# Improbable-AI/walk-these-ways

Measured on NVIDIA H100. Metric: env_steps_per_s, higher is better.
Workload: dtype tf32

## Files before the change

walk-these-ways_b200/csrc/gemm_tf32.cu:

```cuda
#include <cuda_runtime.h>
#include <cuda.h>
#include <cuda_bf16.h>
#include <stdint.h>
#include <stdio.h>
#include <mutex>
#include <unordered_map>
#include <stdlib.h>
#include "../../include/go1_b200.h"
#include "wgmma_tf32.cuh"
#include "activation.cuh"

extern int go1_set_error(const char* m);
void go1_count_launch(int n);

namespace {

constexpr int BM = 128, BK = 32;
constexpr int NCONS = 8, EPI_G = 2;

__device__ __forceinline__ uint32_t smem_u32(const void* p) { return (uint32_t)__cvta_generic_to_shared(p); }

__device__ __forceinline__ void mbar_init(uint64_t* bar, uint32_t count) {
    asm volatile("mbarrier.init.shared::cta.b64 [%0], %1;" ::"r"(smem_u32(bar)), "r"(count));
}
__device__ __forceinline__ void mbar_expect_tx(uint64_t* bar, uint32_t bytes) {
    asm volatile("mbarrier.arrive.expect_tx.shared::cta.b64 _, [%0], %1;" ::"r"(smem_u32(bar)), "r"(bytes) : "memory");
}
__device__ __forceinline__ void mbar_wait(uint64_t* bar, uint32_t parity) {
    uint32_t done = 0;
    const uint32_t a = smem_u32(bar);
    while (!done) {
        asm volatile("{\n\t.reg .pred p;\n\tmbarrier.try_wait.parity.shared::cta.b64 p, [%1], %2;\n\tselp.u32 %0, 1, 0, p;\n\t}"
                     : "=r"(done) : "r"(a), "r"(parity) : "memory");
    }
}
__device__ __forceinline__ void mbar_arrive(uint64_t* bar) {
    asm volatile("mbarrier.arrive.shared::cta.b64 _, [%0];" ::"r"(smem_u32(bar)) : "memory");
}
__device__ __forceinline__ bool elect_one() {
    uint32_t pred = 0;
    asm volatile("{\n\t.reg .pred p;\n\telect.sync _|p, 0xffffffff;\n\tselp.u32 %0, 1, 0, p;\n\t}" : "=r"(pred));
    return pred != 0;
}
__device__ __forceinline__ void tma_load_2d(const CUtensorMap* map, uint64_t* bar, void* dst, int c0, int c1) {
    asm volatile("cp.async.bulk.tensor.2d.shared::cluster.global.mbarrier::complete_tx::bytes [%0], [%1, {%3, %4}], [%2];"
                 ::"r"(smem_u32(dst)), "l"(map), "r"(smem_u32(bar)), "r"(c0), "r"(c1) : "memory");
}
__device__ __forceinline__ void tma_load_2d_multicast(const CUtensorMap* map, uint64_t* bar, void* dst, int c0, int c1, uint16_t cta_mask) {
    asm volatile("cp.async.bulk.tensor.2d.shared::cluster.global.mbarrier::complete_tx::bytes.multicast::cluster [%0], [%1, {%3, %4}], [%2], %5;"
                 ::"r"(smem_u32(dst)), "l"(map), "r"(smem_u32(bar)), "r"(c0), "r"(c1), "h"(cta_mask) : "memory");
}
__device__ __forceinline__ uint32_t cluster_ctarank() {
    uint32_t r;
    asm("mov.u32 %0, %%cluster_ctarank;" : "=r"(r));
    return r;
}
__device__ __forceinline__ void cluster_sync() {
    asm volatile("barrier.cluster.arrive.release;\n\tbarrier.cluster.wait.acquire;" ::: "memory");
}
__device__ __forceinline__ void mbar_arrive_cluster(uint64_t* bar, uint32_t rank) {
    uint32_t remote;
    asm volatile("mapa.shared::cluster.u32 %0, %1, %2;" : "=r"(remote) : "r"(smem_u32(bar)), "r"(rank));
    asm volatile("mbarrier.arrive.shared::cluster.b64 _, [%0];" ::"r"(remote) : "memory");
}
__device__ __forceinline__ void cons_sync() { asm volatile("bar.sync 1, 256;" ::: "memory"); }
__device__ __forceinline__ void wg_sync(int wgi) { asm volatile("bar.sync %0, 128;" ::"r"(2 + wgi) : "memory"); }
__device__ __forceinline__ void fence_async_smem() { asm volatile("fence.proxy.async.shared::cta;" ::: "memory"); }

template <int W>
__device__ __forceinline__ void transpose_tile(const float* __restrict__ raw, uint8_t* dst, const int ctid) {
#pragma unroll
    for (int it = 0; it < W * 8 / 256; it++) {
        const int idx = ctid + 256 * it;
        const int mn = idx % W, kq = idx / W;
        const float* r = raw + (size_t)(4 * kq) * W + mn;
        *reinterpret_cast<float4*>(dst + mn * 128 + ((kq ^ (mn & 7)) << 4)) = make_float4(r[0], r[W], r[2 * W], r[3 * W]);
    }
}

template <int NJ, typename F>
__device__ __forceinline__ void store_fragment(const float (&acc)[4 * NJ], uint8_t* tile, const int col_base, const int w, const int lane, F f) {
    const int rb = 16 * w + (lane >> 2);
#pragma unroll
    for (int j = 0; j < NJ; j++) {
        const int col = col_base + 8 * j + 2 * (lane & 3);
        uint8_t* p = tile + (size_t)(col >> 5) * (64 * 128) + rb * 128 + ((((col & 31) >> 2) ^ (rb & 7)) << 4) + (lane & 1) * 8;
        *reinterpret_cast<float2*>(p) = f(make_float2(acc[4 * j], acc[4 * j + 1]), col, 0);
        *reinterpret_cast<float2*>(p + 8 * 128) = f(make_float2(acc[4 * j + 2], acc[4 * j + 3]), col, 1);
    }
}


struct GemmArgs {
    float* C; const float* bias;
    int M, N, K, ldc, act, kind, accumulate, kb_per_split;
    const float* ex; const float* wex; const float* aux;
    int ldex, ldwex, nex, ldaux;
    int lead;
    int amn, bmn;
    int ct;
    int c16;
    float* colsum;
    const float* bx; const float* bwx; float* gwx; float* dx;
    int ldbx, ldbwx, ldgwx, lddx, nbx;
    int tma_store, tma_aux;
    float* Cg[4]; int nprob, tiles_per_prob;
};
constexpr int GEMM_MAXP = 4;
struct GemmMaps { CUtensorMap a[GEMM_MAXP], b[GEMM_MAXP], half; };

struct EpiStage {
    uint8_t* out;
    const CUtensorMap* mapC;
    const uint8_t* aux;
};
__device__ __forceinline__ void tma_store_2d(const CUtensorMap* map, const void* src, int c0, int c1) {
    asm volatile("cp.async.bulk.tensor.2d.global.shared::cta.bulk_group [%0, {%2, %3}], [%1];"
                 ::"l"(map), "r"(smem_u32(src)), "r"(c0), "r"(c1) : "memory");
}

__device__ __forceinline__ uint32_t pack_bf16x2(float lo, float hi) {
    return (uint32_t)__bfloat16_as_ushort(__float2bfloat16_rn(lo)) | ((uint32_t)__bfloat16_as_ushort(__float2bfloat16_rn(hi)) << 16);
}

template <typename D>
__device__ __forceinline__ void epilogue_dact(const D dact, const GemmArgs& g, float (&v)[32], const int row, const int col0, const int ncols, const int lane,
                                              const float4 (&ypre)[8], const bool have_pre, const EpiStage& es) {
    const float* arow = g.aux + (size_t)row * g.ldaux + col0;
    if (es.aux) {
        const uint8_t* srow = es.aux + lane * 128;
#pragma unroll
        for (int j = 0; j < 8; j++) {
            const float4 y = *reinterpret_cast<const float4*>(srow + ((j ^ (lane & 7)) << 4));
            v[4 * j] *= dact(y.x); v[4 * j + 1] *= dact(y.y); v[4 * j + 2] *= dact(y.z); v[4 * j + 3] *= dact(y.w);
        }
    } else if (have_pre) {
#pragma unroll
        for (int j = 0; j < 8; j++) {
            const float4 y = ypre[j];
            v[4 * j] *= dact(y.x); v[4 * j + 1] *= dact(y.y); v[4 * j + 2] *= dact(y.z); v[4 * j + 3] *= dact(y.w);
        }
    } else if (ncols == 32 && (g.ldaux & 3) == 0 && ((((uintptr_t)g.aux) & 15) == 0) && ((col0 & 3) == 0)) {
#pragma unroll
        for (int j = 0; j < 8; j++) {
            const float4 y = __ldg(reinterpret_cast<const float4*>(arow) + j);
            v[4 * j] *= dact(y.x); v[4 * j + 1] *= dact(y.y); v[4 * j + 2] *= dact(y.z); v[4 * j + 3] *= dact(y.w);
        }
    } else {
#pragma unroll
        for (int j = 0; j < 32; j++) if (j < ncols) v[j] *= dact(__ldg(arow + j));
    }
}
// ... 56 lines not shown
            wl[t] = (t < g.nex && lead_j) ? __ldg(g.wex + (size_t)cj * g.ldwex + t) : 0.f;
        }
        if (g.nex <= 2) {
#pragma unroll
            for (int j = 0; j < 32; j++)
                v[j] += fmaf(e[1], __shfl_sync(0xffffffffu, wl[1], j), e[0] * __shfl_sync(0xffffffffu, wl[0], j));
        } else {
#pragma unroll
            for (int j = 0; j < 32; j++) {
                float a = e[0] * __shfl_sync(0xffffffffu, wl[0], j);
                a = fmaf(e[1], __shfl_sync(0xffffffffu, wl[1], j), a);
                a = fmaf(e[2], __shfl_sync(0xffffffffu, wl[2], j), a);
                v[j] += fmaf(e[3], __shfl_sync(0xffffffffu, wl[3], j), a);
            }
        }
    }
    if (g.bias) {
        const float bl = cj < g.N ? __ldg(g.bias + cj) : 0.f;
#pragma unroll
        for (int j = 0; j < 32; j++) v[j] += __shfl_sync(0xffffffffu, bl, j);
    }
    const int kind = ANYKIND ? g.kind : (int)GO1_ACT_ELU;
    if (row_ok) {
    if (g.act == 1) {
        const int nlead = g.lead <= 0 ? 32 : max(0, min(32, g.lead - col0));
        GO1_ACT_SWITCH(kind, KD,
            _Pragma("unroll")
            for (int j = 0; j < 32; j++) if (j < nlead) v[j] = act_fast<KD>(v[j]);)
    } else if (g.act == 2) {
        if (ANYKIND) epilogue_dact(act_deriv_coefficients(kind), g, v, row, col0, ncols, lane, ypre, have_pre, es);
        else epilogue_dact([](float y) { return act_deriv<GO1_ACT_ELU>(y); }, g, v, row, col0, ncols, lane, ypre, have_pre, es);
    }
    }
    if (g.colsum) {
        float sred[32];
#pragma unroll
        for (int j = 0; j < 32; j++) sred[j] = (row_ok && j < ncols) ? v[j] : 0.f;
        const float s = transpose_reduce32(sred, lane);
        if (lane < ncols) atomicAdd(g.colsum + col0 + lane, s);
    }
    if (g.nbx > 0) {
        const int cjx = col0 + lane;
#pragma unroll
        for (int t = 0; t < 4; t++) {
            if (t < g.nbx) {
                if (g.gwx) {
                const float e = row_ok ? __ldg(g.bx + (size_t)row * g.ldbx + t) : 0.f;
                float sred[32];
#pragma unroll
                for (int j = 0; j < 32; j++) sred[j] = (row_ok && j < ncols) ? v[j] * e : 0.f;
                const float s = transpose_reduce32(sred, lane);
                if (lane < ncols) atomicAdd(g.gwx + (size_t)cjx * g.ldgwx + t, s);
                }
                if (g.dx) {
                    const float wl = lane < ncols ? __ldg(g.bwx + (size_t)cjx * g.ldbwx + t) : 0.f;
                    float acc = 0.f;
#pragma unroll
                    for (int j = 0; j < 32; j++) acc = fmaf(v[j], __shfl_sync(0xffffffffu, wl, j), acc);
                    if (row_ok) atomicAdd(g.dx + (size_t)row * g.lddx + t, acc);
                }
            }
        }
    }
    if (ROW16 && g.c16 && !g.ct) {
        if (es.out) {
            __syncwarp();
            uint8_t* srow = es.out + lane * 64;
#pragma unroll
            for (int j = 0; j < 4; j++) {
                uint4 o;
                o.x = pack_bf16x2(v[8 * j], v[8 * j + 1]); o.y = pack_bf16x2(v[8 * j + 2], v[8 * j + 3]);
                o.z = pack_bf16x2(v[8 * j + 4], v[8 * j + 5]); o.w = pack_bf16x2(v[8 * j + 6], v[8 * j + 7]);
                *reinterpret_cast<uint4*>(srow + ((j ^ ((lane >> 1) & 3)) << 4)) = o;
            }
            asm volatile("fence.proxy.async.shared::cta;" ::: "memory");
            __syncwarp();
            if (lane == 0) {
                tma_store_2d(es.mapC, es.out, col0, row);
                asm volatile("cp.async.bulk.commit_group;" ::: "memory");
            }
        } else if (row_ok) {
            uint16_t* c16 = reinterpret_cast<uint16_t*>(Cbase) + (size_t)row * g.ldc + col0;
#pragma unroll
            for (int j = 0; j < 32; j++) if (j < ncols) c16[j] = __bfloat16_as_ushort(__float2bfloat16_rn(v[j]));
        }
        return;
    }
    if (es.out) {
        if (g.ct && g.c16) {
            __syncwarp();
#pragma unroll
            for (int j = 0; j < 32; j++) *reinterpret_cast<__nv_bfloat16*>(es.out + j * 64 + lane * 2) = __float2bfloat16_rn(v[j]);
        } else if (g.ct) {
            __syncwarp();
#pragma unroll
            for (int j = 0; j < 32; j++)
                *reinterpret_cast<float*>(es.out + j * 128 + ((((lane >> 2) ^ (j & 7)) << 4) | ((lane & 3) << 2))) = v[j];
        } else {
            uint8_t* srow = es.out + lane * 128;
#pragma unroll
            for (int j = 0; j < 8; j++)
                *reinterpret_cast<float4*>(srow + ((j ^ (lane & 7)) << 4)) = make_float4(v[4 * j], v[4 * j + 1], v[4 * j + 2], v[4 * j + 3]);
        }
        asm volatile("fence.proxy.async.shared::cta;" ::: "memory");
        __syncwarp();
        if (lane == 0) {
            if (g.ct) tma_store_2d(es.mapC, es.out, row, col0);
            else tma_store_2d(es.mapC, es.out, col0, row);
            asm volatile("cp.async.bulk.commit_group;" ::: "memory");
        }
        return;
    }
    if (!row_ok) return;
    if (vec) {
#pragma unroll
        for (int j = 0; j < 8; j++) reinterpret_cast<float4*>(crow)[j] = make_float4(v[4 * j], v[4 * j + 1], v[4 * j + 2], v[4 * j + 3]);
    } else {
#pragma unroll
        for (int j = 0; j < 32; j++) if (j < ncols) crow[j] = v[j];
    }
}

__device__ __forceinline__ bool epilogue_prefetch(const GemmArgs& g, const int row, const int col0, const bool split, float4 (&ypre)[8]) {
    if (g.act != 2 || split || col0 + 32 > g.N || (g.ldaux & 3) != 0 || ((((uintptr_t)g.aux) & 15) != 0) || (col0 & 3) != 0) return false;
    const float4* arow = reinterpret_cast<const float4*>(g.aux + (size_t)(row < g.M ? row : 0) * g.ldaux + col0);
#pragma unroll
    for (int j = 0; j < 8; j++) ypre[j] = __ldg(arow + j);
    return true;
}

constexpr int X_BYTES = 65536;
template <int BN, bool ANYKIND, int CL, bool BF16, int AMN, int BMN, bool ROW16>
__device__ __forceinline__ void gemm_wgmma_body(const GemmMaps& gm, const CUtensorMap& mapC, const CUtensorMap& mapY, const GemmArgs& g,
                                                const int tiles_m, const int tiles_n, const int total_tiles, const int stages) {
    static_assert(CL == 1 || (CL == 2 && BN == BM), "CTA pairs share 128-row operand boxes");
// ... 592 lines not shown
    const size_t smem = L::TOTAL;
    static bool configured = false;
    if (!configured) {
        cudaError_t e = cudaFuncSetAttribute(mlp_tail_fwd_ragged_kernel<N2, N3, ANYKIND>, cudaFuncAttributeMaxDynamicSharedMemorySize, (int)smem);
        if (e != cudaSuccess) return go1_set_error(cudaGetErrorString(e));
        configured = true;
    }
    const int sms = sm_count();
    const int grid = g.tiles < sms ? g.tiles : sms;
    mlp_tail_fwd_ragged_kernel<N2, N3, ANYKIND><<<grid, 32 * NCONS + 128, smem, st>>>(maps, g, d);
    go1_count_launch(1);
    return 0;
}

template <bool ANYKIND>
int launch_tail_ragged_any(const TailMaps& maps, const TailArgs& g, const TailDims d, cudaStream_t st) {
    const int w2 = d.n2 <= 64 ? 64 : d.n2 <= 128 ? 128 : 256, w3 = d.n3 == 0 ? 0 : d.n3 <= 64 ? 64 : d.n3 <= 128 ? 128 : -1;
#define GO1_TAIL_CASE(A, B) if (w2 == A && w3 == B) return launch_tail_ragged<A, B, ANYKIND>(maps, g, d, st);
    GO1_TAIL_CASE(64, 0) GO1_TAIL_CASE(64, 64) GO1_TAIL_CASE(64, 128)
    GO1_TAIL_CASE(128, 0) GO1_TAIL_CASE(128, 64) GO1_TAIL_CASE(128, 128)
    GO1_TAIL_CASE(256, 0) GO1_TAIL_CASE(256, 64) GO1_TAIL_CASE(256, 128)
#undef GO1_TAIL_CASE
    return go1_set_error("go1_mlp_tail_forward: tail widths N2 1..256, N3 0..128");
}

}

#include <vector>
static bool g_time_on = false;
static std::vector<cudaEvent_t> g_time_events;
static size_t g_time_used = 0;
static double g_time_flop = 0.0;
struct TimeRec { int M, N, K, amn, bmn, act, nex, splits, kern, colsum, cluster, n3, heads, problems, bf16; };
static std::vector<TimeRec> g_time_recs;
static cudaEvent_t timing_event() {
    if (g_time_used == g_time_events.size()) { cudaEvent_t e; cudaEventCreate(&e); g_time_events.push_back(e); }
    return g_time_events[g_time_used++];
}
extern "C" int go1_gemm_timing(int on, double* total_ms, double* total_flop, long long* launches) {
    if (on) { g_time_on = true; g_time_used = 0; g_time_flop = 0.0; g_time_recs.clear(); return 0; }
    g_time_on = false;
    double ms = 0.0;
    FILE* csv = getenv("GO1_GEMM_TIMING_CSV") ? fopen(getenv("GO1_GEMM_TIMING_CSV"), "w") : nullptr;
    if (csv) fprintf(csv, "M,N,K,a_mn_major,b_mn_major,act,num_extra,splits,kernel,colsum,us,n3,heads,problems,bf16\n");
    for (size_t i = 0; i + 1 < g_time_used; i += 2) {
        if (cudaEventSynchronize(g_time_events[i + 1]) != cudaSuccess) return go1_set_error("go1_gemm_timing: event sync failed");
        float t = 0.f;
        if (cudaEventElapsedTime(&t, g_time_events[i], g_time_events[i + 1]) != cudaSuccess) return go1_set_error("go1_gemm_timing: elapsed time failed");
        ms += t;
        if (csv && i / 2 < g_time_recs.size()) {
            const TimeRec& r = g_time_recs[i / 2];
            fprintf(csv, "%d,%d,%d,%d,%d,%d,%d,%d,%s,%d,%.2f,%d,%d,%d,%d\n", r.M, r.N, r.K, r.amn, r.bmn, r.act, r.nex, r.splits,
                    r.kern >= 1000 ? (r.kern == 1003 ? "tail3" : "tail2") : (r.kern == 128 ? (r.cluster == 2 ? "p128c2" : "p128") : (r.kern == 64 ? "p64" : "p32")),
                    r.colsum, 1e3 * t, r.n3, r.heads, r.problems, r.bf16);
        }
    }
    if (csv) fclose(csv);
    if (total_ms) *total_ms = ms;
    if (total_flop) *total_flop = g_time_flop;
    if (launches) *launches = (long long)(g_time_used / 2);
    return 0;
}

template <int BN, bool ANYKIND>
int launch_gemm_mn(int mn, const GemmMaps& gm, const CUtensorMap& mc, const CUtensorMap& my, GemmArgs& g, int splits, cudaStream_t st) {
    switch (mn) {
        case 0: return launch_gemm<BN, ANYKIND, 1, true, 0>(gm, mc, my, g, splits, st);
        case 1: return launch_gemm<BN, ANYKIND, 1, true, 1>(gm, mc, my, g, splits, st);
        case 2: return launch_gemm<BN, ANYKIND, 1, true, 2>(gm, mc, my, g, splits, st);
        default: return launch_gemm<BN, ANYKIND, 1, true, 3>(gm, mc, my, g, splits, st);
    }
}

template <typename T>
static int gemm_wgmma_impl(int transA, int transB, int M, int N, int K, int nprob, const T* const* As, int lda, const T* const* Bs, int ldb,
                           float* const* Cs, int ldc, const Go1GemmEpilogue* ep, cudaStream_t st, bool mn = false, bool row16 = false) {
    constexpr bool BF16 = sizeof(T) == 2;
    constexpr int ES = sizeof(T), KE = 128 / ES;
    float* Cm = Cs[0];
    const float* bias = ep->bias; const int act = ep->act, accumulate = ep->accumulate;
    if (act < 0 || act > 2) return go1_set_error("go1_gemm_ex: act must be 0, 1 or 2");
    if (!go1_act_kind_ok(ep->act_kind)) return go1_set_error("go1_gemm_ex: unknown activation kind (Go1Activation)");
    const int amn = transA ? 1 : 0, bmn = transB ? 0 : 1;
    if (BF16 && !mn && (amn || bmn)) return go1_set_error("go1_gemm_bf16_ex: both operands must be K-major (transA = 0, transB = 1)");
    const bool c16 = ep->out_bf16 != nullptr;
    if (row16 && (c16 || ep->store_transposed || accumulate || nprob != 1 || (ldc & 7) || ldc < N || (((uintptr_t)Cm) & 15)))
        return go1_set_error("go1_gemm_bf16_mn: c_bf16 needs a 16-byte aligned C with ldc >= N, a multiple of 8, no accumulate, no store_transposed and no out_bf16");
    if (c16 && (!ep->store_transposed || (ep->ld_out_bf16 & 7) || ep->ld_out_bf16 < M || (((uintptr_t)ep->out_bf16) & 15)))
        return go1_set_error("go1_gemm_ex: out_bf16 needs store_transposed, a 16-byte aligned output and ld_out_bf16 >= M, a multiple of 8");
    for (int p = 0; p < nprob; p++)
        if (((lda * ES) & 15) || ((ldb * ES) & 15) || (((uintptr_t)As[p] | (uintptr_t)Bs[p]) & 15) || (!Cs[p] && !c16))
            return go1_set_error(BF16 ? (mn ? "go1_gemm_bf16_mn: A/B must be 16-byte aligned with row strides that are multiples of 8 elements (TMA)"
                                            : "go1_gemm_bf16_ex: A/B must be 16-byte aligned with row strides that are multiples of 8 elements (TMA)")
                                      : "go1_gemm impl=1: A/B must be 16-byte aligned with row strides that are multiples of 4 floats (TMA)");
    GemmArgs g;
    g.nprob = nprob; g.tiles_per_prob = 0;
    for (int p = 0; p < GEMM_MAXP; p++) g.Cg[p] = Cs[p < nprob ? p : 0];
    g.C = Cm; g.bias = bias; g.M = M; g.N = N; g.K = K; g.ldc = ldc; g.act = act; g.kind = ep->act_kind; g.accumulate = accumulate;
    g.ex = ep->extra; g.ldex = ep->ld_extra; g.wex = ep->w_extra; g.ldwex = ep->ld_w_extra; g.nex = ep->extra ? ep->num_extra : 0;
    g.aux = ep->dact_y; g.ldaux = ep->ld_dact_y;
    g.amn = amn; g.bmn = bmn; g.lead = ep->lead_cols; g.colsum = ep->colsum; g.ct = ep->store_transposed ? 1 : 0; g.c16 = (c16 || row16) ? 1 : 0;
    g.nbx = ep->num_bwd_extra; g.bx = ep->bwd_extra; g.bwx = ep->bwd_w_extra; g.gwx = ep->g_w_extra; g.dx = ep->d_extra;
    g.ldbx = ep->ld_bwd_extra; g.ldbwx = ep->ld_bwd_w_extra; g.ldgwx = ep->ld_g_w_extra; g.lddx = ep->ld_d_extra;
    if (g.nbx < 0 || g.nbx > 4 || (g.nbx > 0 && ((g.gwx && !g.bx) || (!g.gwx && !g.dx) || (g.dx && !g.bwx)))) return go1_set_error("go1_gemm_ex: bad fused trailing-input backward arguments");
    if (g.nex < 0 || g.nex > 4) return go1_set_error("go1_gemm_ex: num_extra must be 0..4");
    if (act == 2 && !g.aux) return go1_set_error("go1_gemm_ex: act 2 needs dact_y");
    if (g.ct && (nprob != 1 || accumulate || M < 32 || (!c16 && ((ldc & 3) || (((uintptr_t)Cm) & 15)))))
        return go1_set_error("go1_gemm_ex: store_transposed needs M >= 32, no accumulate and a 16-byte aligned C with ldc a multiple of 4");
    const int num_kb = (K + KE - 1) / KE;
    constexpr int SPLIT_MIN_KB = 16;
    const int BN = (N > 64) ? 128 : (N > 32 ? 64 : 32);
    const int tiles = ((M + BM - 1) / BM) * ((N + BN - 1) / BN) * nprob;
    const bool plain = g.nex == 0 && act != 2 && g.lead <= 0 && !g.colsum && g.nbx == 0 && !g.ct && !row16;
    const int splits = plain ? split_count(tiles, num_kb, SPLIT_MIN_KB, sm_count()) : 1;
    g.kb_per_split = (num_kb + splits - 1) / splits;
    GemmMaps gm;
    for (int p = 0; p < nprob; p++) {
        int e = 0;
        if (BF16 && amn) e = make_map(&gm.a[p], As[p], K, M, lda, KE, BM / 2, CU_TENSOR_MAP_SWIZZLE_128B, ES);
        else e = amn ? make_map_mn(&gm.a[p], (const float*)As[p], K, M, lda, BM) : make_map(&gm.a[p], As[p], M, K, lda, BM, KE, CU_TENSOR_MAP_SWIZZLE_128B, ES);
        if (e) return e;
        if (BF16 && bmn) e = make_map(&gm.b[p], Bs[p], K, N, ldb, KE, BN == 32 ? 32 : 64, BN == 32 ? CU_TENSOR_MAP_SWIZZLE_64B : CU_TENSOR_MAP_SWIZZLE_128B, ES);
        else e = bmn ? make_map_mn(&gm.b[p], (const float*)Bs[p], K, N, ldb, BN) : make_map(&gm.b[p], Bs[p], N, K, ldb, BN, KE, CU_TENSOR_MAP_SWIZZLE_128B, ES);
        if (e) return e;
    }
    const int mnk = BF16 && (amn || bmn || row16) ? (amn | (bmn << 1)) : -1;
    for (int p = nprob; p < GEMM_MAXP; p++) { gm.a[p] = gm.a[0]; gm.b[p] = gm.b[0]; }
    const CUtensorMap& ma = gm.a[0];
    const int tiles_m = (M + BM - 1) / BM, tiles_n = (N + BN - 1) / BN;
    const int cluster = (mnk < 0 && !amn && !bmn && nprob == 1 && act != 2 && BN == 128 && (tiles_n % 2 == 0 || tiles_m % 2 == 0)) ? 2 : 1;
    gm.half = ma;
    if (cluster == 2) {
        if (int e = tiles_n % 2 == 0 ? make_map(&gm.half, As[0], M, K, lda, BM / 2, KE, CU_TENSOR_MAP_SWIZZLE_128B, ES)
                                     : make_map(&gm.half, Bs[0], N, K, ldb, BN / 2, KE, CU_TENSOR_MAP_SWIZZLE_128B, ES)) return e;
    }
    if (splits > 1) {
        if (!accumulate)
            for (int p = 0; p < nprob; p++) { const size_t tot = (size_t)M * N; zero_strided<<<(unsigned)((tot + 255) / 256), 256, 0, st>>>(Cs[p], ldc, M, N); go1_count_launch(1); }
        g.bias = nullptr; g.act = 0;
    }
    cudaStreamCaptureStatus cap = cudaStreamCaptureStatusNone;
    const bool timed = g_time_on && cudaStreamIsCapturing(st, &cap) == cudaSuccess && cap == cudaStreamCaptureStatusNone;
    if (timed) {
        cudaEventRecord(timing_event(), st); g_time_flop += 2.0 * (double)M * (double)N * (double)K * nprob;
        g_time_recs.push_back({M * nprob, N, K, amn, bmn, act, g.nex, splits, BN, g.colsum ? 1 : 0, cluster, 0, 0, nprob, BF16 ? (mn ? 2 : 1) : 0});
    }
    int e;
    CUtensorMap mc = ma, my = ma;
    g.tma_store = g.tma_aux = 0;
    if (row16) {
        if (N >= 32) {
            if (int e2 = make_map(&mc, Cm, M, N, ldc, 32, 32, CU_TENSOR_MAP_SWIZZLE_64B, 2)) return e2;
            g.tma_store = 1;
        }
    } else if (c16) {
        if (int e2 = make_map(&mc, ep->out_bf16, N, M, ep->ld_out_bf16, 32, 32, CU_TENSOR_MAP_SWIZZLE_NONE, 2)) return e2;
        g.tma_store = 1;
    } else if (nprob == 1 && splits == 1 && !accumulate && (g.ct ? M : N) >= 32 && (ldc & 3) == 0 && (((uintptr_t)Cm) & 15) == 0) {
        if (int e2 = g.ct ? make_map(&mc, Cm, N, M, ldc, 32) : make_map(&mc, Cm, M, N, ldc, 32)) return e2;
        g.tma_store = 1;
    }
    if (g.tma_store) {
        if (g.act == 2 && (g.ldaux & 3) == 0 && (((uintptr_t)g.aux) & 15) == 0) {
            if (int e2 = make_map(&my, g.aux, M, N, g.ldaux, 32)) return e2;
            g.tma_aux = 1;
        }
    }
    const bool any = g.act != 0 && g.kind != GO1_ACT_ELU;
    if (mnk >= 0) {
        if (BN == 128) e = any ? launch_gemm_mn<128, true>(mnk, gm, mc, my, g, splits, st) : launch_gemm_mn<128, false>(mnk, gm, mc, my, g, splits, st);
        else if (BN == 64) e = any ? launch_gemm_mn<64, true>(mnk, gm, mc, my, g, splits, st) : launch_gemm_mn<64, false>(mnk, gm, mc, my, g, splits, st);
        else e = any ? launch_gemm_mn<32, true>(mnk, gm, mc, my, g, splits, st) : launch_gemm_mn<32, false>(mnk, gm, mc, my, g, splits, st);
    } else if (cluster == 2) e = any ? launch_gemm<128, true, 2, BF16>(gm, mc, my, g, splits, st) : launch_gemm<128, false, 2, BF16>(gm, mc, my, g, splits, st);
    else if (BN == 128) e = any ? launch_gemm<128, true, 1, BF16>(gm, mc, my, g, splits, st) : launch_gemm<128, false, 1, BF16>(gm, mc, my, g, splits, st);
    else if (BN == 64) e = any ? launch_gemm<64, true, 1, BF16>(gm, mc, my, g, splits, st) : launch_gemm<64, false, 1, BF16>(gm, mc, my, g, splits, st);
    else e = any ? launch_gemm<32, true, 1, BF16>(gm, mc, my, g, splits, st) : launch_gemm<32, false, 1, BF16>(gm, mc, my, g, splits, st);
    if (e) return e;
    if (splits > 1 && (bias || act))
// ... 128 lines not shown
```

Before: 1.669 million.

## Add persistent weight-stationary dgrad kernel for small-K activation-backward GEMMs

Adds a specialized TF32 wgmma kernel for the backward data-gradient GEMM (act==2, small K up to 256). Each CTA keeps its full W column slice resident in shared memory, transposed once, and streams 64-row dz tiles through two producer rings. It applies the activation derivative from TMA-loaded y tiles and fuses colsum, the trailing-input dx and the transposed store. This removes repeated W loads and split/epilogue overhead of the general kernel. The trade-offs are a more complex routing path and fixed 64x64 tiles that may underuse the tensor cores compared with the 128-row kernel.

Result: faster. 1.732 million (median of 6 runs) (+3.8%).

```diff
diff --git a/walk-these-ways_b200/csrc/gemm_dgrad.cu b/walk-these-ways_b200/csrc/gemm_dgrad.cu
--- /dev/null
+++ b/walk-these-ways_b200/csrc/gemm_dgrad.cu
@@ -0,0 +1,250 @@
+#include <cuda_runtime.h>
+#include <cuda.h>
+#include <stdint.h>
+#include "../../include/go1_b200.h"
+#include "wgmma_tf32.cuh"
+#include "tma_sm90.cuh"
+#include "activation.cuh"
+#include "gemm_dgrad.h"
+
+extern int go1_set_error(const char* m);
+void go1_count_launch(int n);
+
+namespace {
+
+constexpr int BM = DGRAD_BM, BK = 32, NCONS = 8, MAX_STAGES = 8;
+constexpr int A_BYTES = BM * BK * 4;
+constexpr int BN = DGRAD_BN;
+constexpr int YWG = BM * BN * 4;
+constexpr int MAX_YB = 4;
+constexpr int WKB = BN * BK * 4;
+static_assert(DGRAD_MAX_K / BK * WKB <= 2 * 2 * YWG, "the raw W boxes are staged in the y_prev buffers");
+
+__device__ __forceinline__ void bulk_wait_read0() { asm volatile("cp.async.bulk.wait_group.read 0;" ::: "memory"); }
+
+template <bool ANYKIND>
+__global__ void __launch_bounds__(32 * NCONS + 96, 1) dgrad_tf32_wgmma(const __grid_constant__ DgradMaps maps, const DgradArgs g,
+                                                                       const int tiles_n, const int c, const int stages, const int nyb) {
+    extern __shared__ __align__(1024) uint8_t smem_raw[];
+    uint8_t* base = (uint8_t*)(((uintptr_t)smem_raw + 1023) & ~(uintptr_t)1023);
+    const int nkb = (g.K + BK - 1) / BK;
+    uint8_t* wsl = base;
+    uint8_t* stg = wsl + (size_t)nkb * WKB;
+    uint8_t* ring = stg + (size_t)nyb * 2 * YWG;
+    float* s_bw = (float*)(ring + (size_t)2 * stages * A_BYTES);
+    float* s_cs = s_bw + BN * 4;
+    uint64_t* full = (uint64_t*)(s_cs + BN);
+    uint64_t* empty = full + 2 * MAX_STAGES;
+    uint64_t* yfull = empty + 2 * MAX_STAGES;
+    uint64_t* yfree = yfull + 2 * MAX_YB;
+    uint64_t* wfull = yfree + 2 * MAX_YB;
+    uint64_t* wready = wfull + 1;
+
+    const int warp = threadIdx.x >> 5, lane = threadIdx.x & 31;
+    const int n0 = (int)(blockIdx.x % tiles_n) * BN, j0 = (int)blockIdx.x / tiles_n;
+    const int tiles_m = (g.M + BM - 1) / BM;
+
+    if (threadIdx.x == 0) {
+        asm volatile("prefetch.tensormap [%0];" ::"l"(&maps.a) : "memory");
+        asm volatile("prefetch.tensormap [%0];" ::"l"(&maps.w) : "memory");
+        asm volatile("prefetch.tensormap [%0];" ::"l"(&maps.y) : "memory");
+        asm volatile("prefetch.tensormap [%0];" ::"l"(&maps.c) : "memory");
+        for (int w = 0; w < 2; w++)
+            for (int s = 0; s < stages; s++) { mbar_init(&full[w * MAX_STAGES + s], 1); mbar_init(&empty[w * MAX_STAGES + s], NCONS / 2); }
+        for (int b = 0; b < 2 * nyb; b++) { mbar_init(&yfull[b], 1); mbar_init(&yfree[b], 1); }
+        mbar_init(wfull, 1); mbar_init(wready, 1);
+        asm volatile("fence.mbarrier_init.release.cluster;" ::: "memory");
+    }
+    for (int i = threadIdx.x; i < BN * 4; i += blockDim.x) {
+        const int n = i >> 2, t = i & 3;
+        s_bw[i] = (t < g.nbx && n0 + n < g.N) ? __ldg(g.bwx + (size_t)(n0 + n) * g.ldbwx + t) : 0.f;
+    }
+    for (int i = threadIdx.x; i < BN; i += blockDim.x) s_cs[i] = 0.f;
+    __syncthreads();
+
+    if (warp == NCONS || warp == NCONS + 1) {
+        const int p = warp - NCONS;
+        uint8_t* rp = ring + (size_t)p * stages * A_BYTES;
+        uint64_t* fp = full + p * MAX_STAGES;
+        uint64_t* ep = empty + p * MAX_STAGES;
+        if (elect_one()) {
+            int s = 0, ph = 0;
+            for (int tm = j0 + p * c; tm < tiles_m; tm += 2 * c) {
+                for (int kb = 0; kb < nkb; kb++) {
+                    mbar_wait(&ep[s], ph ^ 1);
+                    mbar_expect_tx(&fp[s], A_BYTES);
+                    tma_load_2d(&maps.a, &fp[s], rp + (size_t)s * A_BYTES, kb * BK, tm * BM);
+                    if (++s == stages) { s = 0; ph ^= 1; }
+                }
+            }
+        }
+        return;
+    }
+    if (warp == NCONS + 2) {
+        if (elect_one()) {
+            mbar_expect_tx(wfull, nkb * WKB);
+            for (int kb = 0; kb < nkb; kb++) tma_load_2d(&maps.w, wfull, stg + (size_t)kb * WKB, n0, kb * BK);
+            mbar_wait(wready, 0);
+            for (int tm = j0, i = 0; tm < tiles_m; tm += c, i++) {
+                const int k = i >> 1, yb = 2 * (k % nyb) + (i & 1);
+                mbar_wait(&yfree[yb], ((k / nyb) & 1) ^ 1);
+                uint32_t bytes = 0;
+                for (int cc = 0; cc < BN / 32; cc++) bytes += n0 + 32 * cc < g.N ? BM * 128 : 0;
+                mbar_expect_tx(&yfull[yb], bytes);
+                for (int cc = 0; cc < BN / 32; cc++)
+                    if (n0 + 32 * cc < g.N) tma_load_2d(&maps.y, &yfull[yb], stg + (size_t)yb * YWG + cc * (BM * 128), n0 + 32 * cc, tm * BM);
+            }
+        }
+        return;
+    }
+
+    const int wgi = warp >> 2, w = warp & 3, ctid = threadIdx.x;
+    const bool leader = w == 0 && lane == 0;
+    const int rq = 16 * w + (lane >> 2), q = lane & 3;
+    mbar_wait(wfull, 0);
+    for (int kb = 0; kb < nkb; kb++) transpose_tile<BN>((const float*)(stg + (size_t)kb * WKB), wsl + (size_t)kb * WKB, ctid);
+    fence_async_smem();
+    cons_sync();
+    if (ctid == 0) mbar_arrive(wready);
+
+    const ActDeriv dk = act_deriv_coefficients(ANYKIND ? g.kind : (int)GO1_ACT_ELU);
+    auto dact = [&](float y) { if constexpr (ANYKIND) return dk(y); else return act_deriv<GO1_ACT_ELU>(y); };
+    float cs[BN / 4];
+#pragma unroll
+    for (int k = 0; k < BN / 4; k++) cs[k] = 0.f;
+    uint8_t* rw = ring + (size_t)wgi * stages * A_BYTES;
+    uint64_t* fw = full + wgi * MAX_STAGES;
+    uint64_t* ew = empty + wgi * MAX_STAGES;
+    auto release = [&](int st) { if (lane == 0) mbar_arrive(&ew[st]); };
+    int s = 0, ph = 0;
+    for (int tm = j0 + wgi * c, k = 0; tm < tiles_m; tm += 2 * c, k++) {
+        const int m0 = tm * BM, b = k % nyb;
+        if (k > 0 && leader) { bulk_wait_read0(); mbar_arrive(&yfree[2 * ((k - 1) % nyb) + wgi]); }
+        float acc[BN / 2];
+        int prev = -1;
+        for (int kb = 0; kb < nkb; kb++) {
+            mbar_wait(&fw[s], ph);
+            wg::fence();
+            wg::mma_kblock<BN>(acc, rw + (size_t)s * A_BYTES, wsl + (size_t)kb * WKB, kb > 0);
+            wg::commit();
+            if (prev >= 0) { wg::wait<1>(); release(prev); }
+            prev = s;
+            if (++s == stages) { s = 0; ph ^= 1; }
+        }
+        wg::wait<0>();
+        release(prev);
+        mbar_wait(&yfull[2 * b + wgi], (k / nyb) & 1);
+        uint8_t* yb = stg + (size_t)(2 * b + wgi) * YWG;
+#pragma unroll
+        for (int j = 0; j < BN / 8; j++) {
+            const int col = 8 * j + 2 * q;
+            if (n0 + 32 * (j >> 2) < g.N) {
+                const uint8_t* p = yb + (j >> 2) * (BM * 128) + rq * 128 + ((((col & 31) >> 2) ^ (rq & 7)) << 4) + (q & 1) * 8;
+                const float2 y0 = *reinterpret_cast<const float2*>(p), y1 = *reinterpret_cast<const float2*>(p + 1024);
+                acc[4 * j] *= dact(y0.x); acc[4 * j + 1] *= dact(y0.y); acc[4 * j + 2] *= dact(y1.x); acc[4 * j + 3] *= dact(y1.y);
+            }
+            cs[2 * j] += acc[4 * j] + acc[4 * j + 2];
+            cs[2 * j + 1] += acc[4 * j + 1] + acc[4 * j + 3];
+        }
+        if (g.nbx > 0) {
+            float d[2][4] = {};
+#pragma unroll
+            for (int j = 0; j < BN / 8; j++) {
+                const float4 wa = *reinterpret_cast<const float4*>(s_bw + (8 * j + 2 * q) * 4), wb = *reinterpret_cast<const float4*>(s_bw + (8 * j + 2 * q + 1) * 4);
+                d[0][0] = fmaf(acc[4 * j], wa.x, fmaf(acc[4 * j + 1], wb.x, d[0][0])); d[1][0] = fmaf(acc[4 * j + 2], wa.x, fmaf(acc[4 * j + 3], wb.x, d[1][0]));
+                d[0][1] = fmaf(acc[4 * j], wa.y, fmaf(acc[4 * j + 1], wb.y, d[0][1])); d[1][1] = fmaf(acc[4 * j + 2], wa.y, fmaf(acc[4 * j + 3], wb.y, d[1][1]));
+                d[0][2] = fmaf(acc[4 * j], wa.z, fmaf(acc[4 * j + 1], wb.z, d[0][2])); d[1][2] = fmaf(acc[4 * j + 2], wa.z, fmaf(acc[4 * j + 3], wb.z, d[1][2]));
+                d[0][3] = fmaf(acc[4 * j], wa.w, fmaf(acc[4 * j + 1], wb.w, d[0][3])); d[1][3] = fmaf(acc[4 * j + 2], wa.w, fmaf(acc[4 * j + 3], wb.w, d[1][3]));
+            }
+#pragma unroll
+            for (int r = 0; r < 2; r++)
+#pragma unroll
+                for (int t = 0; t < 4; t++) {
+                    d[r][t] += __shfl_xor_sync(0xffffffffu, d[r][t], 1);
+                    d[r][t] += __shfl_xor_sync(0xffffffffu, d[r][t], 2);
+                }
+            if (q < g.nbx) {
+                const float v0 = q == 0 ? d[0][0] : q == 1 ? d[0][1] : q == 2 ? d[0][2] : d[0][3];
+                const float v1 = q == 0 ? d[1][0] : q == 1 ? d[1][1] : q == 2 ? d[1][2] : d[1][3];
+                if (m0 + rq < g.M) atomicAdd(g.dx + (size_t)(m0 + rq) * g.lddx + q, v0);
+                if (m0 + rq + 8 < g.M) atomicAdd(g.dx + (size_t)(m0 + rq + 8) * g.lddx + q, v1);
+            }
+        }
+        if (g.ct) {
+            wg_sync(wgi);
+#pragma unroll
+            for (int j = 0; j < BN / 8; j++)
+#pragma unroll
+                for (int e = 0; e < 4; e++) {
+                    const int row = rq + 8 * (e >> 1), n = 8 * j + 2 * q + (e & 1);
+                    *reinterpret_cast<float*>(yb + (row >> 5) * (BN * 128) + n * 128 + ((((row & 31) >> 2) ^ (n & 7)) << 4) + (row & 3) * 4) = acc[4 * j + e];
+                }
+        } else {
+#pragma unroll
+            for (int j = 0; j < BN / 8; j++) {
+                const int col = 8 * j + 2 * q;
+                uint8_t* p = yb + (j >> 2) * (BM * 128) + rq * 128 + ((((col & 31) >> 2) ^ (rq & 7)) << 4) + (q & 1) * 8;
+                *reinterpret_cast<float2*>(p) = make_float2(acc[4 * j], acc[4 * j + 1]);
+                *reinterpret_cast<float2*>(p + 1024) = make_float2(acc[4 * j + 2], acc[4 * j + 3]);
+            }
+        }
+        fence_async_smem();
+        wg_sync(wgi);
+        if (leader) {
+            if (g.ct) {
+                for (int h = 0; h < 2; h++) if (m0 + 32 * h < g.M) tma_store_2d(&maps.c, yb + h * (BN * 128), m0 + 32 * h, n0);
+            } else {
+                for (int cc = 0; cc < BN / 32; cc++) if (n0 + 32 * cc < g.N) tma_store_2d(&maps.c, yb + cc * (BM * 128), n0 + 32 * cc, m0);
+            }
+            asm volatile("cp.async.bulk.commit_group;" ::: "memory");
+        }
+    }
+    if (leader) asm volatile("cp.async.bulk.wait_group 0;" ::: "memory");
+    if (g.colsum) {
+#pragma unroll
+        for (int k = 0; k < BN / 4; k++) {
+            cs[k] += __shfl_xor_sync(0xffffffffu, cs[k], 4);
+            cs[k] += __shfl_xor_sync(0xffffffffu, cs[k], 8);
+            cs[k] += __shfl_xor_sync(0xffffffffu, cs[k], 16);
+        }
+        if (lane < 4) {
+#pragma unroll
+            for (int j = 0; j < BN / 8; j++) { atomicAdd(&s_cs[8 * j + 2 * q], cs[2 * j]); atomicAdd(&s_cs[8 * j + 2 * q + 1], cs[2 * j + 1]); }
+        }
+        cons_sync();
+        if (ctid < BN && n0 + ctid < g.N) atomicAdd(g.colsum + n0 + ctid, s_cs[ctid]);
+    }
+}
+
+}
+
+int launch_dgrad(const DgradMaps& maps, const DgradArgs& g, int sms, cudaStream_t st) {
+    if (g.K < 1 || g.K > DGRAD_MAX_K) return go1_set_error("dgrad_tf32_wgmma: K must be 1..256");
+    const int nkb = (g.K + BK - 1) / BK;
+    const size_t budget = 227 * 1024;
+    int nyb = MAX_YB, stages = 0;
+    size_t fixed = 0;
+    for (;; nyb--) {
+        fixed = (size_t)nkb * WKB + (size_t)nyb * 2 * YWG + (BN * 4 + BN) * 4 + (4 * MAX_YB + 4 * MAX_STAGES + 2) * 8 + 1024;
+        stages = (int)((budget - fixed) / (2 * A_BYTES));
+        if (stages >= (nkb < 6 ? nkb : 6) || nyb == 2) break;
+    }
+    if (stages > MAX_STAGES) stages = MAX_STAGES;
+    if (stages < 2) return go1_set_error("dgrad_tf32_wgmma: no room for the dz rings");
+    const size_t smem = fixed + (size_t)2 * stages * A_BYTES;
+    const bool any = g.kind != GO1_ACT_ELU;
+    auto kernel = any ? dgrad_tf32_wgmma<true> : dgrad_tf32_wgmma<false>;
+    static bool configured[2] = {false, false};
+    if (!configured[any]) {
+        cudaError_t e = cudaFuncSetAttribute(kernel, cudaFuncAttributeMaxDynamicSharedMemorySize, (int)budget);
+        if (e != cudaSuccess) return go1_set_error(cudaGetErrorString(e));
+        configured[any] = true;
+    }
+    const int tiles_m = (g.M + BM - 1) / BM, tiles_n = (g.N + BN - 1) / BN;
+    int c = sms / tiles_n;
+    if (c < 1) c = 1;
+    if (c > tiles_m) c = tiles_m;
+    kernel<<<tiles_n * c, 32 * NCONS + 96, smem, st>>>(maps, g, tiles_n, c, stages, nyb);
+    go1_count_launch(1);
+    return 0;
+}
diff --git a/walk-these-ways_b200/csrc/gemm_dgrad.h b/walk-these-ways_b200/csrc/gemm_dgrad.h
--- /dev/null
+++ b/walk-these-ways_b200/csrc/gemm_dgrad.h
@@ -0,0 +1,19 @@
+#pragma once
+#include <cuda.h>
+#include <cuda_runtime.h>
+
+struct DgradArgs {
+    int M, N, K, kind;
+    int ct;
+    float* colsum;
+    const float* bwx;
+    float* dx;
+    int ldbwx, lddx, nbx;
+};
+struct DgradMaps { CUtensorMap a, w, y, c; };
+
+constexpr int DGRAD_BM = 64;
+constexpr int DGRAD_BN = 64;
+constexpr int DGRAD_MAX_K = 256;
+
+int launch_dgrad(const DgradMaps& maps, const DgradArgs& g, int sms, cudaStream_t st);
diff --git a/walk-these-ways_b200/csrc/gemm_tf32.cu b/walk-these-ways_b200/csrc/gemm_tf32.cu
--- a/walk-these-ways_b200/csrc/gemm_tf32.cu
+++ b/walk-these-ways_b200/csrc/gemm_tf32.cu
@@ -8,7 +8,9 @@
 #include <stdlib.h>
 #include "../../include/go1_b200.h"
 #include "wgmma_tf32.cuh"
+#include "tma_sm90.cuh"
 #include "activation.cuh"
+#include "gemm_dgrad.h"
 
 extern int go1_set_error(const char* m);
 void go1_count_launch(int n);
@@ -18,34 +20,6 @@
 constexpr int BM = 128, BK = 32;
 constexpr int NCONS = 8, EPI_G = 2;
 
-__device__ __forceinline__ uint32_t smem_u32(const void* p) { return (uint32_t)__cvta_generic_to_shared(p); }
-
-__device__ __forceinline__ void mbar_init(uint64_t* bar, uint32_t count) {
-    asm volatile("mbarrier.init.shared::cta.b64 [%0], %1;" ::"r"(smem_u32(bar)), "r"(count));
-}
-__device__ __forceinline__ void mbar_expect_tx(uint64_t* bar, uint32_t bytes) {
-    asm volatile("mbarrier.arrive.expect_tx.shared::cta.b64 _, [%0], %1;" ::"r"(smem_u32(bar)), "r"(bytes) : "memory");
-}
-__device__ __forceinline__ void mbar_wait(uint64_t* bar, uint32_t parity) {
-    uint32_t done = 0;
-    const uint32_t a = smem_u32(bar);
-    while (!done) {
-        asm volatile("{\n\t.reg .pred p;\n\tmbarrier.try_wait.parity.shared::cta.b64 p, [%1], %2;\n\tselp.u32 %0, 1, 0, p;\n\t}"
-                     : "=r"(done) : "r"(a), "r"(parity) : "memory");
-    }
-}
-__device__ __forceinline__ void mbar_arrive(uint64_t* bar) {
-    asm volatile("mbarrier.arrive.shared::cta.b64 _, [%0];" ::"r"(smem_u32(bar)) : "memory");
-}
-__device__ __forceinline__ bool elect_one() {
-    uint32_t pred = 0;
-    asm volatile("{\n\t.reg .pred p;\n\telect.sync _|p, 0xffffffff;\n\tselp.u32 %0, 1, 0, p;\n\t}" : "=r"(pred));
-    return pred != 0;
-}
-__device__ __forceinline__ void tma_load_2d(const CUtensorMap* map, uint64_t* bar, void* dst, int c0, int c1) {
-    asm volatile("cp.async.bulk.tensor.2d.shared::cluster.global.mbarrier::complete_tx::bytes [%0], [%1, {%3, %4}], [%2];"
-                 ::"r"(smem_u32(dst)), "l"(map), "r"(smem_u32(bar)), "r"(c0), "r"(c1) : "memory");
-}
 __device__ __forceinline__ void tma_load_2d_multicast(const CUtensorMap* map, uint64_t* bar, void* dst, int c0, int c1, uint16_t cta_mask) {
     asm volatile("cp.async.bulk.tensor.2d.shared::cluster.global.mbarrier::complete_tx::bytes.multicast::cluster [%0], [%1, {%3, %4}], [%2], %5;"
                  ::"r"(smem_u32(dst)), "l"(map), "r"(smem_u32(bar)), "r"(c0), "r"(c1), "h"(cta_mask) : "memory");
@@ -63,21 +37,6 @@
     asm volatile("mapa.shared::cluster.u32 %0, %1, %2;" : "=r"(remote) : "r"(smem_u32(bar)), "r"(rank));
     asm volatile("mbarrier.arrive.shared::cluster.b64 _, [%0];" ::"r"(remote) : "memory");
 }
-__device__ __forceinline__ void cons_sync() { asm volatile("bar.sync 1, 256;" ::: "memory"); }
-__device__ __forceinline__ void wg_sync(int wgi) { asm volatile("bar.sync %0, 128;" ::"r"(2 + wgi) : "memory"); }
-__device__ __forceinline__ void fence_async_smem() { asm volatile("fence.proxy.async.shared::cta;" ::: "memory"); }
-
-template <int W>
-__device__ __forceinline__ void transpose_tile(const float* __restrict__ raw, uint8_t* dst, const int ctid) {
-#pragma unroll
-    for (int it = 0; it < W * 8 / 256; it++) {
-        const int idx = ctid + 256 * it;
-        const int mn = idx % W, kq = idx / W;
-        const float* r = raw + (size_t)(4 * kq) * W + mn;
-        *reinterpret_cast<float4*>(dst + mn * 128 + ((kq ^ (mn & 7)) << 4)) = make_float4(r[0], r[W], r[2 * W], r[3 * W]);
-    }
-}
-
 template <int NJ, typename F>
 __device__ __forceinline__ void store_fragment(const float (&acc)[4 * NJ], uint8_t* tile, const int col_base, const int w, const int lane, F f) {
     const int rb = 16 * w + (lane >> 2);
@@ -114,10 +73,6 @@
     const CUtensorMap* mapC;
     const uint8_t* aux;
 };
-__device__ __forceinline__ void tma_store_2d(const CUtensorMap* map, const void* src, int c0, int c1) {
-    asm volatile("cp.async.bulk.tensor.2d.global.shared::cta.bulk_group [%0, {%2, %3}], [%1];"
-                 ::"l"(map), "r"(smem_u32(src)), "r"(c0), "r"(c1) : "memory");
-}
 
 __device__ __forceinline__ uint32_t pack_bf16x2(float lo, float hi) {
     return (uint32_t)__bfloat16_as_ushort(__float2bfloat16_rn(lo)) | ((uint32_t)__bfloat16_as_ushort(__float2bfloat16_rn(hi)) << 16);
@@ -967,6 +922,7 @@
 static size_t g_time_used = 0;
 static double g_time_flop = 0.0;
 struct TimeRec { int M, N, K, amn, bmn, act, nex, splits, kern, colsum, cluster, n3, heads, problems, bf16; };
+constexpr int TIME_DGRAD = 2000;
 static std::vector<TimeRec> g_time_recs;
 static cudaEvent_t timing_event() {
     if (g_time_used == g_time_events.size()) { cudaEvent_t e; cudaEventCreate(&e); g_time_events.push_back(e); }
@@ -985,8 +941,10 @@
         ms += t;
         if (csv && i / 2 < g_time_recs.size()) {
             const TimeRec& r = g_time_recs[i / 2];
+            char dg[16];
+            snprintf(dg, sizeof dg, "dg%d", r.kern - TIME_DGRAD);
             fprintf(csv, "%d,%d,%d,%d,%d,%d,%d,%d,%s,%d,%.2f,%d,%d,%d,%d\n", r.M, r.N, r.K, r.amn, r.bmn, r.act, r.nex, r.splits,
-                    r.kern >= 1000 ? (r.kern == 1003 ? "tail3" : "tail2") : (r.kern == 128 ? (r.cluster == 2 ? "p128c2" : "p128") : (r.kern == 64 ? "p64" : "p32")),
+                    r.kern >= TIME_DGRAD ? dg : r.kern >= 1000 ? (r.kern == 1003 ? "tail3" : "tail2") : (r.kern == 128 ? (r.cluster == 2 ? "p128c2" : "p128") : (r.kern == 64 ? "p64" : "p32")),
                     r.colsum, 1e3 * t, r.n3, r.heads, r.problems, r.bf16);
         }
     }
@@ -1042,6 +1000,30 @@
     if (act == 2 && !g.aux) return go1_set_error("go1_gemm_ex: act 2 needs dact_y");
     if (g.ct && (nprob != 1 || accumulate || M < 32 || (!c16 && ((ldc & 3) || (((uintptr_t)Cm) & 15)))))
         return go1_set_error("go1_gemm_ex: store_transposed needs M >= 32, no accumulate and a 16-byte aligned C with ldc a multiple of 4");
+    if constexpr (!BF16) {
+        const bool dgrad = !amn && bmn && nprob == 1 && act == 2 && !bias && g.nex == 0 && g.lead <= 0 && !accumulate && !c16 &&
+                           K <= DGRAD_MAX_K && M >= 64 && N >= 32 && (g.nbx == 0 || !g.gwx) && (g.ldaux & 3) == 0 && (((uintptr_t)g.aux) & 15) == 0 &&
+                           (ldc & 3) == 0 && (((uintptr_t)Cm) & 15) == 0;
+        if (dgrad) {
+            DgradMaps dm;
+            if (int e = make_map(&dm.a, As[0], M, K, lda, DGRAD_BM)) return e;
+            if (int e = make_map_mn(&dm.w, Bs[0], K, N, ldb, DGRAD_BN)) return e;
+            if (int e = make_map(&dm.y, g.aux, M, N, g.ldaux, DGRAD_BM)) return e;
+            if (int e = g.ct ? make_map(&dm.c, Cm, N, M, ldc, DGRAD_BN) : make_map(&dm.c, Cm, M, N, ldc, DGRAD_BM)) return e;
+            const DgradArgs da = {M, N, K, ep->act_kind, g.ct, g.colsum, g.bwx, g.dx, g.ldbwx, g.lddx, g.nbx};
+            cudaStreamCaptureStatus cap = cudaStreamCaptureStatusNone;
+            const bool timed = g_time_on && cudaStreamIsCapturing(st, &cap) == cudaSuccess && cap == cudaStreamCaptureStatusNone;
+            if (timed) {
+                cudaEventRecord(timing_event(), st); g_time_flop += 2.0 * (double)M * (double)N * (double)K;
+                g_time_recs.push_back({M, N, K, amn, bmn, act, 0, 1, TIME_DGRAD + DGRAD_BN, g.colsum ? 1 : 0, 1, 0, 0, 1, 0});
+            }
+            if (int e = launch_dgrad(dm, da, sm_count(), st)) return e;
+            if (timed) cudaEventRecord(timing_event(), st);
+            cudaError_t ce = cudaGetLastError();
+            if (ce != cudaSuccess) return go1_set_error(cudaGetErrorString(ce));
+            return 0;
+        }
+    }
     const int num_kb = (K + KE - 1) / KE;
     constexpr int SPLIT_MIN_KB = 16;
     const int BN = (N > 64) ? 128 : (N > 32 ? 64 : 32);
diff --git a/walk-these-ways_b200/csrc/tma_sm90.cuh b/walk-these-ways_b200/csrc/tma_sm90.cuh
--- /dev/null
+++ b/walk-these-ways_b200/csrc/tma_sm90.cuh
@@ -0,0 +1,54 @@
+#pragma once
+#include <cuda.h>
+#include <stdint.h>
+
+namespace {
+
+__device__ __forceinline__ uint32_t smem_u32(const void* p) { return (uint32_t)__cvta_generic_to_shared(p); }
+
+__device__ __forceinline__ void mbar_init(uint64_t* bar, uint32_t count) {
+    asm volatile("mbarrier.init.shared::cta.b64 [%0], %1;" ::"r"(smem_u32(bar)), "r"(count));
+}
+__device__ __forceinline__ void mbar_expect_tx(uint64_t* bar, uint32_t bytes) {
+    asm volatile("mbarrier.arrive.expect_tx.shared::cta.b64 _, [%0], %1;" ::"r"(smem_u32(bar)), "r"(bytes) : "memory");
+}
+__device__ __forceinline__ void mbar_wait(uint64_t* bar, uint32_t parity) {
+    uint32_t done = 0;
+    const uint32_t a = smem_u32(bar);
+    while (!done) {
+        asm volatile("{\n\t.reg .pred p;\n\tmbarrier.try_wait.parity.shared::cta.b64 p, [%1], %2;\n\tselp.u32 %0, 1, 0, p;\n\t}"
+                     : "=r"(done) : "r"(a), "r"(parity) : "memory");
+    }
+}
+__device__ __forceinline__ void mbar_arrive(uint64_t* bar) {
+    asm volatile("mbarrier.arrive.shared::cta.b64 _, [%0];" ::"r"(smem_u32(bar)) : "memory");
+}
+__device__ __forceinline__ bool elect_one() {
+    uint32_t pred = 0;
+    asm volatile("{\n\t.reg .pred p;\n\telect.sync _|p, 0xffffffff;\n\tselp.u32 %0, 1, 0, p;\n\t}" : "=r"(pred));
+    return pred != 0;
+}
+__device__ __forceinline__ void tma_load_2d(const CUtensorMap* map, uint64_t* bar, void* dst, int c0, int c1) {
+    asm volatile("cp.async.bulk.tensor.2d.shared::cluster.global.mbarrier::complete_tx::bytes [%0], [%1, {%3, %4}], [%2];"
+                 ::"r"(smem_u32(dst)), "l"(map), "r"(smem_u32(bar)), "r"(c0), "r"(c1) : "memory");
+}
+__device__ __forceinline__ void tma_store_2d(const CUtensorMap* map, const void* src, int c0, int c1) {
+    asm volatile("cp.async.bulk.tensor.2d.global.shared::cta.bulk_group [%0, {%2, %3}], [%1];"
+                 ::"l"(map), "r"(smem_u32(src)), "r"(c0), "r"(c1) : "memory");
+}
+__device__ __forceinline__ void cons_sync() { asm volatile("bar.sync 1, 256;" ::: "memory"); }
+__device__ __forceinline__ void wg_sync(int wgi) { asm volatile("bar.sync %0, 128;" ::"r"(2 + wgi) : "memory"); }
+__device__ __forceinline__ void fence_async_smem() { asm volatile("fence.proxy.async.shared::cta;" ::: "memory"); }
+
+template <int W>
+__device__ __forceinline__ void transpose_tile(const float* __restrict__ raw, uint8_t* dst, const int ctid) {
+#pragma unroll
+    for (int it = 0; it < W * 8 / 256; it++) {
+        const int idx = ctid + 256 * it;
+        const int mn = idx % W, kq = idx / W;
+        const float* r = raw + (size_t)(4 * kq) * W + mn;
+        *reinterpret_cast<float4*>(dst + mn * 128 + ((kq ^ (mn & 7)) << 4)) = make_float4(r[0], r[W], r[2 * W], r[3 * W]);
+    }
+}
+
+}
```

## Stage column sums through shared tile and transpose dgrad weights to K-major

Applied to the files above, without the earlier changes.

The column-sum reduction now reads values back from the already-staged shared-memory output tile instead of doing a register transpose-reduce, in the non-transposed fp32 TMA-store path. Separately, for eager-mode tf32 dgrad GEMMs with an MN-major weight and small K, the weight is transposed into a pooled temporary buffer so the main GEMM reads a K-major B operand. The goal is to replace shuffle-heavy reductions and a slower MN-major operand path, at the cost of an extra transpose launch, a pool allocation and a smem readback.

Measured after the change: 1.659 million before, 1.680 million after, median of 6. 1.3% higher.

```diff
diff --git a/walk-these-ways_b200/csrc/gemm_tf32.cu b/walk-these-ways_b200/csrc/gemm_tf32.cu
--- a/walk-these-ways_b200/csrc/gemm_tf32.cu
+++ b/walk-these-ways_b200/csrc/gemm_tf32.cu
@@ -240,7 +240,8 @@
         else epilogue_dact([](float y) { return act_deriv<GO1_ACT_ELU>(y); }, g, v, row, col0, ncols, lane, ypre, have_pre, es);
     }
     }
-    if (g.colsum) {
+    const bool sum_staged = !ANYKIND && !ROW16 && g.colsum && es.out && !g.ct && !g.c16;
+    if (g.colsum && !sum_staged) {
         float sred[32];
 #pragma unroll
         for (int j = 0; j < 32; j++) sred[j] = (row_ok && j < ncols) ? v[j] : 0.f;
@@ -295,6 +296,10 @@
         return;
     }
     if (es.out) {
+        if (sum_staged) {
+#pragma unroll
+            for (int j = 0; j < 32; j++) v[j] = (row_ok && j < ncols) ? v[j] : 0.f;
+        }
         if (g.ct && g.c16) {
             __syncwarp();
 #pragma unroll
@@ -309,6 +314,13 @@
 #pragma unroll
             for (int j = 0; j < 8; j++)
                 *reinterpret_cast<float4*>(srow + ((j ^ (lane & 7)) << 4)) = make_float4(v[4 * j], v[4 * j + 1], v[4 * j + 2], v[4 * j + 3]);
+        }
+        if (sum_staged) {
+            __syncwarp();
+            float s = 0.f;
+#pragma unroll
+            for (int r = 0; r < 32; r++) s += *reinterpret_cast<const float*>(es.out + r * 128 + ((((lane >> 2) ^ (r & 7)) << 4) | ((lane & 3) << 2)));
+            if (lane < ncols) atomicAdd(g.colsum + col0 + lane, s);
         }
         asm volatile("fence.proxy.async.shared::cta;" ::: "memory");
         __syncwarp();
@@ -1006,6 +1018,37 @@
         default: return launch_gemm<BN, ANYKIND, 1, true, 3>(gm, mc, my, g, splits, st);
     }
 }
+
+__global__ void transpose_kernel(const float* __restrict__ src, int lds, float* __restrict__ dst, int ldd, int rows, int cols);
+
+static cudaMemPool_t weight_copy_pool() {
+    static std::mutex mu;
+    static std::unordered_map<int, cudaMemPool_t> pools;
+    int dev = 0;
+    if (cudaGetDevice(&dev) != cudaSuccess) return nullptr;
+    std::lock_guard<std::mutex> lk(mu);
+    auto it = pools.find(dev);
+    if (it != pools.end()) return it->second;
+    cudaMemPoolProps props = {};
+    props.allocType = cudaMemAllocationTypePinned;
+    props.location.type = cudaMemLocationTypeDevice;
+    props.location.id = dev;
+    cudaMemPool_t pool = nullptr;
+    if (cudaMemPoolCreate(&pool, &props) != cudaSuccess) return nullptr;
+    uint64_t keep = UINT64_MAX;
+    int no = 0;
+    if (cudaMemPoolSetAttribute(pool, cudaMemPoolAttrReleaseThreshold, &keep) != cudaSuccess ||
+        cudaMemPoolSetAttribute(pool, cudaMemPoolReuseAllowInternalDependencies, &no) != cudaSuccess) {
+        cudaMemPoolDestroy(pool);
+        return nullptr;
+    }
+    pools.emplace(dev, pool);
+    return pool;
+}
+struct PoolBlock {
+    void* p; cudaStream_t st;
+    ~PoolBlock() { if (p) cudaFreeAsync(p, st); }
+};
 
 template <typename T>
 static int gemm_wgmma_impl(int transA, int transB, int M, int N, int K, int nprob, const T* const* As, int lda, const T* const* Bs, int ldb,
@@ -1075,10 +1118,26 @@
         g.bias = nullptr; g.act = 0;
     }
     cudaStreamCaptureStatus cap = cudaStreamCaptureStatusNone;
-    const bool timed = g_time_on && cudaStreamIsCapturing(st, &cap) == cudaSuccess && cap == cudaStreamCaptureStatusNone;
+    const bool eager = cudaStreamIsCapturing(st, &cap) == cudaSuccess && cap == cudaStreamCaptureStatusNone;
+    const bool timed = g_time_on && eager;
     if (timed) {
         cudaEventRecord(timing_event(), st); g_time_flop += 2.0 * (double)M * (double)N * (double)K * nprob;
         g_time_recs.push_back({M * nprob, N, K, amn, bmn, act, g.nex, splits, BN, g.colsum ? 1 : 0, cluster, 0, 0, nprob, BF16 ? (mn ? 2 : 1) : 0});
+    }
+    PoolBlock wt{nullptr, st};
+    if (!BF16 && nprob == 1 && bmn && !amn && act == 2 && K >= 32 && K <= 256 && eager) {
+        const int ldt = (K + 3) & ~3;
+        cudaMemPool_t pool = weight_copy_pool();
+        if (!pool || cudaMallocFromPoolAsync(&wt.p, (size_t)N * ldt * 4, pool, st) != cudaSuccess) {
+            wt.p = nullptr;
+            cudaGetLastError();
+            return go1_set_error("go1_gemm impl=1: no memory for the K-major weight copy of a dgrad");
+        }
+        transpose_kernel<<<dim3((N + 31) / 32, (K + 31) / 32), dim3(32, 8), 0, st>>>((const float*)Bs[0], ldb, (float*)wt.p, ldt, K, N);
+        go1_count_launch(1);
+        if (int e2 = make_map(&gm.b[0], wt.p, N, K, ldt, BN)) return e2;
+        for (int p = 1; p < GEMM_MAXP; p++) gm.b[p] = gm.b[0];
+        g.bmn = 0;
     }
     int e;
     CUtensorMap mc = ma, my = ma;
```
